# Huangying-Zhan/DF-VO

Hardware: AMD Instinct MI355X
Metric: KITTI-odom frames/sec (DF-VO per-pair tracking hot path: monodepth2 + LiteFlowNet fwd/bwd + kp selection + E/H RANSAC + scale) (higher is better)
Workload: dtype f32 (f16x3 split products: two f16 planes per operand = 22 mantissa bits, three exact products per term, fp32 accumulate; direct one- / two-channel heads exact fp32)

## Files before the change

df-vo_amd/csrc/conv_gemm_f16s.h:

```cpp
#pragma once

static inline uint32_t f16g_entry(int ky, int kx, int valid, int src, int choff) {
    return (uint32_t)ky | ((uint32_t)kx << 5) | ((uint32_t)valid << 10) | ((uint32_t)src << 11) | ((uint32_t)choff << 16);
}

typedef unsigned int u32x4 __attribute__((ext_vector_type(4)));
typedef __attribute__((address_space(4))) const u32x4 cu32x4;

template <int WP, int KSP, int TC, int PF = 3, bool RAG = false, int NP = 3>
__global__ __launch_bounds__(64 * WP * KSP) void conv_gemm_f16s_kernel(const ConvParams p) {
    extern __shared__ __attribute__((aligned(16))) float f16g_red[];

    const int t = threadIdx.x, lane = t & 63;
    const int wave = __builtin_amdgcn_readfirstlane(t >> 6);
    const int wp = wave / KSP, wk = wave % KSP;
    const int lp = lane & 31, kb = lane >> 5;
    const int M = p.N * p.Ho * p.Wo;
    const int nb = gridDim.x;
    int bid = blockIdx.x;
    {
        const int q = nb >> 3, r = nb & 7, xcd = bid & 7, k = bid >> 3;
        bid = (xcd < r ? xcd * (q + 1) : r * (q + 1) + (xcd - r) * q) + k;
    }
    const int ny = p.wf16g_cout_pad / (32 * TC);
    const int ytile = bid % ny;
    bid /= ny;
    const int m = (bid * WP + wp) * 32 + lp;
    const bool vm = m < M;
    int iy0, ix0, nimg;
    {
        const int mm = vm ? m : 0;
        nimg = mm / (p.Ho * p.Wo);
        const int rem = mm - nimg * (p.Ho * p.Wo);
        const int oy = rem / p.Wo, ox = rem - oy * p.Wo;
        iy0 = oy * p.stride - p.pad_h;
        ix0 = ox * p.stride - p.pad_w;
    }
    const int n0 = ytile * (32 * TC);
    const int S = p.f16g_steps;
    const int per = (S + KSP - 1) / KSP;
    const int s0 = wk * per < S ? wk * per : S;
    const int s1 = s0 + per < S ? s0 + per : S;

    auto pin = [](int v) { return __builtin_amdgcn_readfirstlane(v); };
    auto pin64 = [](unsigned long long v) {
        const unsigned lo = __builtin_amdgcn_readfirstlane((unsigned)v), hi = __builtin_amdgcn_readfirstlane((unsigned)(v >> 32));
        return ((unsigned long long)hi << 32) | lo;
    };
    const cu32x4* const tab = (const cu32x4*)pin64((unsigned long long)p.f16g_tab);
    const unsigned long long src0 = pin64((unsigned long long)p.src0), src1 = pin64((unsigned long long)(p.G1 ? p.src1 : p.src0));
    const int cs0 = pin(p.cs0), cs1 = pin(p.cs1), co0 = pin(p.co0), co1 = pin(p.co1), up0 = pin(p.up0);
    const int H = pin(p.H), W = pin(p.W), refl = pin(p.pad_mode == PAD_REFLECT ? 1 : 0);
    const int H0 = H >> up0, W0 = W >> up0;
    const unsigned short* const wbase = p.wf16g + ((size_t)n0 * 32 + (kb * 32 + lp) * 8);
    const size_t w_step_stride = (size_t)pin(p.wf16g_cout_pad) * 32;

    f32x4 ra[PF][2];
    unsigned rav = 0;
    h16x8 rw[PF][TC][2];
    const bool fast_addr = !refl && up0 == 0;
    int* const gtab = reinterpret_cast<int*>(f16g_red + (KSP > 1 ? WP * KSP * TC * 16 * 64 : 0));
    if (fast_addr) {
        for (int i = t; i < S * 4; i += 64 * WP * KSP) {
            const unsigned e = p.f16g_tab[i];
            const int ky = e & 31, kx = (e >> 5) & 31;
            const bool s1e = ((e >> 11) & 1u) != 0;
            gtab[2 * i] = (ky * W + kx) * (s1e ? cs1 : cs0) + (int)(e >> 16);
            gtab[2 * i + 1] = (int)(e & 0xfffu);
        }
        __syncthreads();
    }
    const int pbase0 = ((nimg * H + iy0) * W + ix0) * cs0 + co0, pbase1 = ((nimg * H + iy0) * W + ix0) * cs1 + co1;
    int nl = s0;
    u32x4 tq = tab[nl < S ? nl : S - 1];
    u32x4 gq = {0u, 0u, 0u, 0u};
    if (fast_addr) gq = *reinterpret_cast<const u32x4*>(gtab + ((nl < S ? nl : S - 1) * 4 + 2 * kb) * 2);
    auto load_step = [&](int st) {
        const int sN = nl + 1 < S ? nl + 1 : S - 1;
        if (fast_addr) {
            const u32x4 gc = gq;
            gq = *reinterpret_cast<const u32x4*>(gtab + (sN * 4 + 2 * kb) * 2);
#pragma unroll
            for (int j = 0; j < 2; ++j) {
                const int d = (int)gc[2 * j];
                const unsigned f = gc[2 * j + 1];
                const int iy = iy0 + (int)(f & 31u), ix = ix0 + (int)((f >> 5) & 31u);
                const bool s1v = ((f >> 11) & 1u) != 0;
                const bool v = vm && ((f >> 10) & 1u) && (unsigned)iy < (unsigned)H && (unsigned)ix < (unsigned)W;
                const int off = v ? (s1v ? pbase1 : pbase0) + d : (s1v ? co1 : co0);
                const unsigned long long base = s1v ? src1 : src0;
                ra[st][j] = *reinterpret_cast<const __attribute__((address_space(1))) f32x4*>(base + (long long)off * 4);
                rav = (rav & ~(1u << (2 * st + j))) | ((v ? 1u : 0u) << (2 * st + j));
            }
        } else {
        const unsigned e0 = __builtin_amdgcn_readfirstlane(tq[0]), e1 = __builtin_amdgcn_readfirstlane(tq[1]),
                       e2 = __builtin_amdgcn_readfirstlane(tq[2]), e3 = __builtin_amdgcn_readfirstlane(tq[3]);
        tq = tab[sN];
#pragma unroll
        for (int j = 0; j < 2; ++j) {
            const unsigned e = kb ? (j ? e3 : e2) : (j ? e1 : e0);
            const int ky = e & 31, kx = (e >> 5) & 31;
            const bool s1v = ((e >> 11) & 1u) != 0;
            int iy = iy0 + ky, ix = ix0 + kx;
            bool v = vm && ((e >> 10) & 1u);
            if (refl) {
                iy = reflect_idx(iy, H);
                ix = reflect_idx(ix, W);
            }
            v = v && iy >= 0 && iy < H && ix >= 0 && ix < W;
            iy = iy < 0 ? 0 : (iy >= H ? H - 1 : iy);
            ix = ix < 0 ? 0 : (ix >= W ? W - 1 : ix);
            const int pix0 = (nimg * H0 + (iy >> up0)) * W0 + (ix >> up0);
            const int pix1 = (nimg * H + iy) * W + ix;
            const int off = (s1v ? pix1 * cs1 + co1 : pix0 * cs0 + co0) + (int)(e >> 16);
            const unsigned long long base = s1v ? src1 : src0;
            ra[st][j] = *reinterpret_cast<const __attribute__((address_space(1))) f32x4*>(base + (long long)off * 4);
            rav = (rav & ~(1u << (2 * st + j))) | ((v ? 1u : 0u) << (2 * st + j));
        }
        }
        const unsigned short* g = wbase + (size_t)nl * w_step_stride;
#pragma unroll
        for (int i = 0; i < TC; ++i) {
            rw[st][i][0] = *reinterpret_cast<const h16x8*>(g + (size_t)i * 1024);
            if constexpr (NP == 3) rw[st][i][1] = *reinterpret_cast<const h16x8*>(g + (size_t)i * 1024 + 512);
        }
        ++nl;
    };

    f32x16 am[TC], ax[TC];
#pragma unroll
    for (int i = 0; i < TC; ++i)
#pragma unroll
        for (int e = 0; e < 16; ++e) am[i][e] = ax[i][e] = 0.f;
    float amax = 0.f;

#pragma unroll
    for (int d = 0; d < PF; ++d)
        if (s0 + d < s1) load_step(d);
    for (int s = s0; s < s1; s += PF) {
#pragma unroll
        for (int u = 0; u < PF; ++u) {
            if (s + u < s1) {
                h16x4 h0, l0 = {}, h1, l1 = {};
                if constexpr (NP == 3) {
                    split_f16_planes(((rav >> (2 * u)) & 1u) ? ra[u][0] : f32x4{0.f, 0.f, 0.f, 0.f}, &h0, &l0, amax);
                    split_f16_planes(((rav >> (2 * u + 1)) & 1u) ? ra[u][1] : f32x4{0.f, 0.f, 0.f, 0.f}, &h1, &l1, amax);
                } else {
                    split_f16_hi(((rav >> (2 * u)) & 1u) ? ra[u][0] : f32x4{0.f, 0.f, 0.f, 0.f}, &h0, amax);
                    split_f16_hi(((rav >> (2 * u + 1)) & 1u) ? ra[u][1] : f32x4{0.f, 0.f, 0.f, 0.f}, &h1, amax);
                }
                const h16x8 xh = __builtin_shufflevector(h0, h1, 0, 1, 2, 3, 4, 5, 6, 7);
                const h16x8 xl = __builtin_shufflevector(l0, l1, 0, 1, 2, 3, 4, 5, 6, 7);
                h16x8 wh[TC], wl[TC];
#pragma unroll
                for (int i = 0; i < TC; ++i) {
                    wh[i] = rw[u][i][0];
                    if constexpr (NP == 3) wl[i] = rw[u][i][1];
                }
                if (s + u + PF < s1) load_step(u);
                if constexpr (NP == 3) {
#pragma unroll
                    for (int i = 0; i < TC; ++i) ax[i] = __builtin_amdgcn_mfma_f32_32x32x16_f16(wh[i], xl, ax[i], 0, 0, 0);
#pragma unroll
                    for (int i = 0; i < TC; ++i) ax[i] = __builtin_amdgcn_mfma_f32_32x32x16_f16(wl[i], xh, ax[i], 0, 0, 0);
                }
#pragma unroll
                for (int i = 0; i < TC; ++i) am[i] = __builtin_amdgcn_mfma_f32_32x32x16_f16(wh[i], xh, am[i], 0, 0, 0);
            }
        }
    }
    f16s_report_clamp(amax);

    if (KSP == 1 && RAG) {
        if (!vm) return;
        float* const drow = p.dst + (size_t)m * p.dst_cs + p.dst_co;
        const float slope = p.act == ACT_LEAKY ? p.act_param : 1.f;
        f32x4 bq[4 * TC];
#pragma unroll
        for (int q = 0; q < 4 * TC; ++q) {
            const int col0 = n0 + (q >> 2) * 32 + 8 * (q & 3) + 4 * kb;
            bq[q] = *reinterpret_cast<const f32x4*>(p.bias + (col0 + 3 < p.cout_pad ? col0 : p.cout_pad - 4));
        }
#pragma unroll
        for (int q = 0; q < 4 * TC; ++q) {
            const int col0 = n0 + (q >> 2) * 32 + 8 * (q & 3) + 4 * kb;
            f32x4 x;
#pragma unroll
            for (int e = 0; e < 4; ++e) {
                const float v = am[q >> 2][4 * (q & 3) + e] + F16S_LO_UNSCALE * ax[q >> 2][4 * (q & 3) + e] + bq[q][e];
                x[e] = (v > 0.f || v != v) ? v : (p.act == ACT_RELU ? 0.f : v * slope);
            }
            if (col0 + 3 < p.cout) {
                *reinterpret_cast<f32x4*>(drow + col0) = x;
            } else {
#pragma unroll
                for (int e = 0; e < 4; ++e) {
                    if (col0 + e < p.cout)
                        drow[col0 + e] = x[e];
                    else if (col0 + e < p.dst_zero_to)
                        drow[col0 + e] = 0.f;
                }
            }
        }
        return;
    }
    if (KSP == 1) {
        ConvEpi<4 * TC> epi;
        conv_epi_init(p, epi, [&](int q) { return n0 + (q >> 2) * 32 + 8 * (q & 3) + 4 * kb; });
        conv_epi_row(p, epi, (size_t)(vm ? m : 0), vm, [&](int q) {
            f32x4 v;
#pragma unroll
            for (int e = 0; e < 4; ++e) v[e] = am[q >> 2][4 * (q & 3) + e] + F16S_LO_UNSCALE * ax[q >> 2][4 * (q & 3) + e];
            return v;
        });
        return;
    }
    float* const mine = f16g_red + (size_t)((wp * KSP + wk) * TC) * 16 * 64;
#pragma unroll
    for (int i = 0; i < TC; ++i)
#pragma unroll
        for (int e = 0; e < 16; ++e) mine[(i * 16 + e) * 64 + lane] = am[i][e] + F16S_LO_UNSCALE * ax[i][e];
    __syncthreads();
    const bool vec_ok = conv_vec_ok(p);
    for (int q = wk; q < 4 * TC; q += KSP) {
        const int i = q >> 2, g = q & 3;
        const int col0 = n0 + i * 32 + 8 * g + 4 * kb;
        const bool fastq = vec_ok && col0 + 3 < p.cout;
        f32x4 b = {0.f, 0.f, 0.f, 0.f}, r = {0.f, 0.f, 0.f, 0.f};
        if (fastq) {
            b = *reinterpret_cast<const f32x4*>(p.bias + col0);
            if (p.res && vm) r = *reinterpret_cast<const f32x4*>(p.res + (size_t)m * p.res_cs + p.res_co + col0);
        }
        f32x4 v = {0.f, 0.f, 0.f, 0.f};
        for (int z = 0; z < KSP; ++z) {
            const float* src = f16g_red + (size_t)((wp * KSP + z) * TC + i) * 16 * 64 + (4 * g) * 64 + lane;
#pragma unroll
            for (int e = 0; e < 4; ++e) v[e] = z == 0 ? src[e * 64] : v[e] + src[e * 64];
        }
        if (!vm) continue;
        if (fastq) {
            f32x4 x = v + b + r;
#pragma unroll
            for (int e = 0; e < 4; ++e) x[e] = apply_act(x[e], p.act, p.act_param);
            *reinterpret_cast<f32x4*>(p.dst + (size_t)m * p.dst_cs + p.dst_co + col0) = x;
        } else {
            conv_epilogue_quad(p, (size_t)m, col0, v, vec_ok);
        }
    }
}

size_t conv_pack_weights_f16g(const float* w, int cout, int c0, int c1, int kh, int kw, const float* fold_scale,
                              unsigned short* out) {
    const int G0 = cdiv(c0, 4), G1 = cdiv(c1, 4), G = G0 + G1, taps = kh * kw;
    const int steps = cdiv(taps * G, 4);
    const int cp = round_up(cout, 32);
    const size_t total = (size_t)steps * cp * 32;
    if (!out) return total;
    memset(out, 0, total * sizeof(unsigned short));
    const int cin = c0 + c1;
    for (int tap = 0; tap < taps; ++tap)
        for (int cg = 0; cg < G; ++cg) {
            const int g = tap * G + cg, step = g >> 2, gl = g & 3;
            for (int q = 0; q < 4; ++q) {
                int ci;
                if (cg < G0) {
                    ci = cg * 4 + q;
                    if (ci >= c0) continue;
                } else {
                    ci = (cg - G0) * 4 + q;
                    if (ci >= c1) continue;
                    ci += c0;
                }
                const int k = gl * 4 + q;
                for (int co = 0; co < cout; ++co) {
                    float v = w[((size_t)co * cin + ci) * taps + tap];
                    if (fold_scale) v *= fold_scale[co];
                    unsigned short* o = out + ((size_t)step * cp + (co & ~31)) * 32 + ((k >> 3) * 32 + (co & 31)) * 8 + (k & 7);
                    f16s_split_host(v, o, o + 512);
                }
            }
        }
    return total;
}

void conv_build_f16g_table(int c0, int c1, int kh, int kw, std::vector<uint32_t>* tab) {
    const int G0 = cdiv(c0, 4), G1 = cdiv(c1, 4), G = G0 + G1, taps = kh * kw;
    const int steps = cdiv(taps * G, 4);
    tab->assign((size_t)steps * 4, f16g_entry(0, 0, 0, 0, 0));
    for (int tap = 0; tap < taps; ++tap)
        for (int cg = 0; cg < G; ++cg)
            (*tab)[(size_t)tap * G + cg] = f16g_entry(tap / kw, tap % kw, 1, cg < G0 ? 0 : 1, cg < G0 ? cg * 4 : (cg - G0) * 4);
}

static bool conv_f16g_ok(const ConvParams& p) {
    if (!p.wf16g || !p.f16g_tab) return false;
    if (p.kh > 31 || p.kw > 31) return false;
    return true;
}

template <int WP, int KSP, int TC, int PF = 3, bool RAG = false>
static int launch_f16g_cfg(const ConvParams& p, hipStream_t stream, int cfg_id) {
    const long long M = (long long)p.N * p.Ho * p.Wo;
    dim3 grid((unsigned)(((M + 32 * WP - 1) / (32 * WP)) * (p.wf16g_cout_pad / (32 * TC))), 1, 1);
    const bool fast_addr = p.pad_mode != PAD_REFLECT && p.up0 == 0;
    const size_t lds = (KSP > 1 ? (size_t)WP * KSP * TC * 16 * 64 * sizeof(float) : 0) + (fast_addr ? (size_t)p.f16g_steps * 32 : 0);
    return with_f16_terms(p, [&](auto np) -> int {
        const auto kernel = conv_gemm_f16s_kernel<WP, KSP, TC, PF, RAG, decltype(np)::value>;
        if (lds > 48 * 1024)
            if (int rc_lds = ensure_dyn_lds((const void*)kernel, lds)) return rc_lds;
        ConvProfScope prof(p, stream, cfg_id);
        hipLaunchKernelGGL(kernel, grid, dim3(64 * WP * KSP), lds, stream, p);
        DFVO_HIP_CHECK(hipGetLastError());
        return prof.done((int)grid.x, TC, KSP * 100 + 1);
    });
}

bool conv_taps_f16s_ok(const ConvParams& p);
int launch_taps_f16s(const ConvParams& p, hipStream_t stream);

static int launch_f16g(const ConvParams& p, hipStream_t stream) {
    const long long M = (long long)p.N * p.Ho * p.Wo;
    const long long mblocks = (M + 31) / 32;
    const int nblk = p.wf16g_cout_pad / 32;
    const long long target = 2048;
    bool tc2 = (nblk % 2) == 0;
    if (tc2 && mblocks * (nblk / 2) * 8 * 2 < target && p.f16g_steps >= 64) tc2 = false;
    const long long tiles = mblocks * (tc2 ? nblk / 2 : nblk);
    int ksp = 1;
    while (ksp < (tc2 ? 8 : 16) && tiles * ksp * 2 <= target && p.f16g_steps >= 4 * ksp * 2) ksp *= 2;
    const int cfg = ksp == 1 ? 20 : 21;
    static const bool taps_on = env_flag("DFVO_TAPS", true);
    if (taps_on && ksp == 1 && conv_taps_f16s_ok(p)) {
        ConvParams pt = p;
        pt.f16s_clamp_ctr = f16s_clamp_counter();
        return launch_taps_f16s(pt, stream);
    }
    const bool rag = ksp == 1 && (p.cout % (tc2 ? 64 : 32)) != 0 && !p.res && ((p.dst_cs | p.dst_co) & 3) == 0 &&
                     p.cout_pad >= 4 && (p.act == ACT_NONE || p.act == ACT_LEAKY || p.act == ACT_RELU);
    if (rag) return tc2 ? launch_f16g_cfg<4, 1, 2, 3, true>(p, stream, cfg) : launch_f16g_cfg<4, 1, 1, 3, true>(p, stream, cfg);
    if (tc2) {
        switch (ksp) {
            case 1: return launch_f16g_cfg<4, 1, 2>(p, stream, cfg);
            case 2: return launch_f16g_cfg<2, 2, 2>(p, stream, cfg);
            case 4: return launch_f16g_cfg<1, 4, 2>(p, stream, cfg);
            default: return launch_f16g_cfg<1, 8, 2>(p, stream, cfg);
        }
    }
    switch (ksp) {
        case 1: return launch_f16g_cfg<4, 1, 1>(p, stream, cfg);
        case 2: return launch_f16g_cfg<2, 2, 1>(p, stream, cfg);
        case 4: return launch_f16g_cfg<1, 4, 1>(p, stream, cfg);
        case 8: return launch_f16g_cfg<1, 8, 1>(p, stream, cfg);
        default: return launch_f16g_cfg<1, 16, 1>(p, stream, cfg);
    }
}
```

Before: 338.1.

## Add persistent resident-grid f16 conv GEMM kernel with weights kept in registers/LDS

Adds a persistent conv GEMM kernel for short-K convolutions (2, 4, or a multiple of 3 steps). It launches a grid sized to a few blocks per CU, and each block loops over output tiles. Weights are loaded once per block into registers (when S is 2 or 4) or into LDS (when S is a multiple of 3 and cout is 32), and the activation prefetch pipeline runs across tile boundaries. This targets the per-block weight reload and launch/tail overhead on layers with small reduction depth and many output pixels. The trade-offs are higher register/LDS pressure, possible load imbalance from the fixed grid, and a simplified epilogue restricted to no-residual and simple activations.

```diff
diff --git a/df-vo_amd/csrc/conv_gemm_f16s.h b/df-vo_amd/csrc/conv_gemm_f16s.h
--- a/df-vo_amd/csrc/conv_gemm_f16s.h
+++ b/df-vo_amd/csrc/conv_gemm_f16s.h
@@ -247,6 +247,188 @@
             conv_epilogue_quad(p, (size_t)m, col0, v, vec_ok);
         }
     }
+}
+
+template <int TC, int PF, bool WREG, int NP>
+__global__ __launch_bounds__(256) void conv_gemm_f16s_res_kernel(const ConvParams p, int tiles) {
+    extern __shared__ __attribute__((aligned(16))) unsigned char f16g_res_lds[];
+    const int t = threadIdx.x, lane = t & 63;
+    const int wave = __builtin_amdgcn_readfirstlane(t >> 6);
+    const int lp = lane & 31, kb = lane >> 5;
+    const int M = p.N * p.Ho * p.Wo;
+    const int S = WREG ? PF : p.f16g_steps;
+    const int ny = p.wf16g_cout_pad / (32 * TC);
+    const int H = p.H, W = p.W, cs0 = p.cs0, co0 = p.co0;
+    auto block_of = [&](int v) {
+        const int q = tiles >> 3, r = tiles & 7, xcd = v & 7, k = v >> 3;
+        return (xcd < r ? xcd * (q + 1) : r * (q + 1) + (xcd - r) * q) + k;
+    };
+    int v = blockIdx.x;
+    const int n0 = (block_of(v) % ny) * (32 * TC);
+
+    int* const gtab = reinterpret_cast<int*>(f16g_res_lds);
+    unsigned char* const wlds = f16g_res_lds + (size_t)S * 32;
+    const unsigned te = t < S * 4 ? p.f16g_tab[t] : 0u;
+    f32x4 bq[4 * TC];
+#pragma unroll
+    for (int q = 0; q < 4 * TC; ++q) {
+        const int col0 = n0 + (q >> 2) * 32 + 8 * (q & 3) + 4 * kb;
+        bq[q] = *reinterpret_cast<const f32x4*>(p.bias + (col0 + 3 < p.cout_pad ? col0 : p.cout_pad - 4));
+    }
+    const unsigned short* const wbase = p.wf16g + ((size_t)n0 * 32 + (kb * 32 + lp) * 8);
+    const size_t w_step_stride = (size_t)p.wf16g_cout_pad * 32;
+    h16x8 rwc[WREG ? PF : 1][TC][2];
+    if constexpr (WREG) {
+#pragma unroll
+        for (int s = 0; s < PF; ++s)
+#pragma unroll
+            for (int i = 0; i < TC; ++i) {
+                rwc[s][i][0] = *reinterpret_cast<const h16x8*>(wbase + s * w_step_stride + (size_t)i * 1024);
+                if constexpr (NP == 3) rwc[s][i][1] = *reinterpret_cast<const h16x8*>(wbase + s * w_step_stride + (size_t)i * 1024 + 512);
+            }
+    } else {
+        const u32x4* const wsrc = reinterpret_cast<const u32x4*>(p.wf16g + (size_t)n0 * 32);
+        const int cps = TC * 128, nchunk = S * cps;
+        const int sstride = p.wf16g_cout_pad * 4;
+        constexpr int WB = 8;
+        for (int c0 = t; c0 < nchunk; c0 += 256 * WB) {
+            u32x4 wv[WB];
+#pragma unroll
+            for (int j = 0; j < WB; ++j) {
+                const int c = c0 + j * 256;
+                if (c < nchunk && (NP == 3 || !((c >> 6) & 1))) wv[j] = wsrc[(size_t)(c / cps) * sstride + (c % cps)];
+            }
+#pragma unroll
+            for (int j = 0; j < WB; ++j) {
+                const int c = c0 + j * 256;
+                if (c < nchunk && (NP == 3 || !((c >> 6) & 1))) *reinterpret_cast<u32x4*>(wlds + (size_t)c * 16) = wv[j];
+            }
+        }
+    }
+    for (int i = t; i < S * 4; i += 256) {
+        const unsigned e = i == t ? te : p.f16g_tab[i];
+        const int ky = e & 31, kx = (e >> 5) & 31;
+        gtab[2 * i] = (ky * W + kx) * cs0 + (int)(e >> 16);
+        gtab[2 * i + 1] = (int)(e & 0xfffu);
+    }
+    __syncthreads();
+
+    int lv = v, ls = 0;
+    bool l_live = true, l_vm = false;
+    int l_iy0 = 0, l_ix0 = 0, l_pbase = 0;
+    auto decode = [&]() {
+        const int m = ((block_of(lv) / ny) * 4 + wave) * 32 + lp;
+        l_vm = m < M;
+        const int mm = l_vm ? m : 0;
+        const int nimg = mm / (p.Ho * p.Wo);
+        const int rem = mm - nimg * (p.Ho * p.Wo);
+        const int oy = rem / p.Wo, ox = rem - oy * p.Wo;
+        l_iy0 = oy * p.stride - p.pad_h;
+        l_ix0 = ox * p.stride - p.pad_w;
+        l_pbase = ((nimg * H + l_iy0) * W + l_ix0) * cs0 + co0;
+    };
+    decode();
+    f32x4 ra[PF][2];
+    unsigned rav = 0;
+    h16x8 rw[WREG ? 1 : PF][TC][2];
+    auto load_step = [&](int st) {
+        if (l_live) {
+            const u32x4 gc = *reinterpret_cast<const u32x4*>(gtab + (ls * 4 + 2 * kb) * 2);
+#pragma unroll
+            for (int j = 0; j < 2; ++j) {
+                const int d = (int)gc[2 * j];
+                const unsigned f = gc[2 * j + 1];
+                const int iy = l_iy0 + (int)(f & 31u), ix = l_ix0 + (int)((f >> 5) & 31u);
+                const bool ok = l_vm && ((f >> 10) & 1u) && (unsigned)iy < (unsigned)H && (unsigned)ix < (unsigned)W;
+                const int off = ok ? l_pbase + d : co0;
+                ra[st][j] = *reinterpret_cast<const f32x4*>(p.src0 + off);
+                rav = (rav & ~(1u << (2 * st + j))) | ((ok ? 1u : 0u) << (2 * st + j));
+            }
+            if constexpr (!WREG) {
+                const unsigned char* g = wlds + (size_t)ls * (TC * 2048) + lane * 16;
+#pragma unroll
+                for (int i = 0; i < TC; ++i) {
+                    rw[st][i][0] = *reinterpret_cast<const h16x8*>(g + i * 2048);
+                    if constexpr (NP == 3) rw[st][i][1] = *reinterpret_cast<const h16x8*>(g + i * 2048 + 1024);
+                }
+            }
+        }
+        if (++ls == S) {
+            ls = 0;
+            lv += (int)gridDim.x;
+            l_live = lv < tiles;
+            if (l_live) decode();
+        }
+    };
+#pragma unroll
+    for (int d = 0; d < PF; ++d) load_step(d);
+
+    const float slope = p.act == ACT_LEAKY ? p.act_param : 1.f;
+    const bool full = (p.cout % (32 * TC)) == 0;
+    float amax = 0.f;
+    for (; v < tiles; v += (int)gridDim.x) {
+        f32x16 am[TC], ax[TC];
+#pragma unroll
+        for (int i = 0; i < TC; ++i)
+#pragma unroll
+            for (int e = 0; e < 16; ++e) am[i][e] = ax[i][e] = 0.f;
+        for (int s = 0; s < S; s += PF) {
+#pragma unroll
+            for (int u = 0; u < PF; ++u) {
+                h16x4 h0, l0 = {}, h1, l1 = {};
+                if constexpr (NP == 3) {
+                    split_f16_planes(((rav >> (2 * u)) & 1u) ? ra[u][0] : f32x4{0.f, 0.f, 0.f, 0.f}, &h0, &l0, amax);
+                    split_f16_planes(((rav >> (2 * u + 1)) & 1u) ? ra[u][1] : f32x4{0.f, 0.f, 0.f, 0.f}, &h1, &l1, amax);
+                } else {
+                    split_f16_hi(((rav >> (2 * u)) & 1u) ? ra[u][0] : f32x4{0.f, 0.f, 0.f, 0.f}, &h0, amax);
+                    split_f16_hi(((rav >> (2 * u + 1)) & 1u) ? ra[u][1] : f32x4{0.f, 0.f, 0.f, 0.f}, &h1, amax);
+                }
+                const h16x8 xh = __builtin_shufflevector(h0, h1, 0, 1, 2, 3, 4, 5, 6, 7);
+                const h16x8 xl = __builtin_shufflevector(l0, l1, 0, 1, 2, 3, 4, 5, 6, 7);
+                h16x8 wh[TC], wl[TC];
+#pragma unroll
+                for (int i = 0; i < TC; ++i) {
+                    wh[i] = WREG ? rwc[WREG ? u : 0][i][0] : rw[WREG ? 0 : u][i][0];
+                    if constexpr (NP == 3) wl[i] = WREG ? rwc[WREG ? u : 0][i][1] : rw[WREG ? 0 : u][i][1];
+                }
+                load_step(u);
+                if constexpr (NP == 3) {
+#pragma unroll
+                    for (int i = 0; i < TC; ++i) ax[i] = __builtin_amdgcn_mfma_f32_32x32x16_f16(wh[i], xl, ax[i], 0, 0, 0);
+#pragma unroll
+                    for (int i = 0; i < TC; ++i) ax[i] = __builtin_amdgcn_mfma_f32_32x32x16_f16(wl[i], xh, ax[i], 0, 0, 0);
+                }
+#pragma unroll
+                for (int i = 0; i < TC; ++i) am[i] = __builtin_amdgcn_mfma_f32_32x32x16_f16(wh[i], xh, am[i], 0, 0, 0);
+            }
+        }
+        const int m = ((block_of(v) / ny) * 4 + wave) * 32 + lp;
+        if (m < M) {
+            float* const drow = p.dst + (size_t)m * p.dst_cs + p.dst_co;
+#pragma unroll
+            for (int q = 0; q < 4 * TC; ++q) {
+                const int col0 = n0 + (q >> 2) * 32 + 8 * (q & 3) + 4 * kb;
+                f32x4 x;
+#pragma unroll
+                for (int e = 0; e < 4; ++e) {
+                    const float r = am[q >> 2][4 * (q & 3) + e] + F16S_LO_UNSCALE * ax[q >> 2][4 * (q & 3) + e] + bq[q][e];
+                    x[e] = (r > 0.f || r != r) ? r : (p.act == ACT_RELU ? 0.f : r * slope);
+                }
+                if (full || col0 + 3 < p.cout) {
+                    *reinterpret_cast<f32x4*>(drow + col0) = x;
+                } else {
+#pragma unroll
+                    for (int e = 0; e < 4; ++e) {
+                        if (col0 + e < p.cout)
+                            drow[col0 + e] = x[e];
+                        else if (col0 + e < p.dst_zero_to)
+                            drow[col0 + e] = 0.f;
+                    }
+                }
+            }
+        }
+    }
+    f16s_report_clamp(amax);
 }
 
 size_t conv_pack_weights_f16g(const float* w, int cout, int c0, int c1, int kh, int kw, const float* fold_scale,
@@ -318,6 +500,53 @@
 bool conv_taps_f16s_ok(const ConvParams& p);
 int launch_taps_f16s(const ConvParams& p, hipStream_t stream);
 
+static int stream_resident_cus() {
+    static int cus[64] = {};
+    int dev = 0;
+    if (hipGetDevice(&dev) != hipSuccess || dev < 0 || dev >= 64) return 256;
+    if (!cus[dev]) {
+        int n = 0;
+        cus[dev] = hipDeviceGetAttribute(&n, hipDeviceAttributeMultiprocessorCount, dev) == hipSuccess && n > 0 ? n : 256;
+    }
+    return cus[dev];
+}
+static int stream_resident_k(int rule_k) {
+    static const int k_env = [] {
+        const char* v = getenv("DFVO_STREAM_RESIDENT_K");
+        return v ? atoi(v) : 0;
+    }();
+    return k_env > 0 ? k_env : rule_k;
+}
+static int f16g_res_pf(const ConvParams& p) {
+    const bool epi_ok = !p.res && ((p.dst_cs | p.dst_co) & 3) == 0 && p.cout_pad >= 4 &&
+                        (p.act == ACT_NONE || p.act == ACT_LEAKY || p.act == ACT_RELU);
+    if (!epi_ok || p.G1 != 0 || p.pad_mode == PAD_REFLECT || p.up0 != 0) return 0;
+    const int S = p.f16g_steps;
+    if (S == 2 || S == 4) return S;
+    if (S % 3 == 0 && p.wf16g_cout_pad == 32 && (size_t)S * (32 + 2048) <= 160 * 1024) return 3;
+    return 0;
+}
+template <int TC, int PF, bool WREG>
+static int launch_f16g_res(const ConvParams& p, hipStream_t stream, int cfg_id) {
+    const long long M = (long long)p.N * p.Ho * p.Wo;
+    const int ny = p.wf16g_cout_pad / (32 * TC);
+    const int tiles = (int)((M + 127) / 128) * ny;
+    const size_t lds = (size_t)p.f16g_steps * 32 + (WREG ? 0 : (size_t)p.f16g_steps * TC * 2048);
+    const int rule_k = p.f16g_steps == 4 ? 1 : 2;
+    int grid = stream_resident_k(rule_k) * stream_resident_cus();
+    grid -= grid % (8 * ny);
+    if (grid >= tiles || grid <= 0) grid = tiles;
+    return with_f16_terms(p, [&](auto np) -> int {
+        const auto kernel = conv_gemm_f16s_res_kernel<TC, PF, WREG, decltype(np)::value>;
+        if (lds > 48 * 1024)
+            if (int rc_lds = ensure_dyn_lds((const void*)kernel, lds)) return rc_lds;
+        ConvProfScope prof(p, stream, cfg_id);
+        hipLaunchKernelGGL(kernel, dim3(grid), dim3(256), lds, stream, p, tiles);
+        DFVO_HIP_CHECK(hipGetLastError());
+        return prof.done(grid, TC, 102);
+    });
+}
+
 static int launch_f16g(const ConvParams& p, hipStream_t stream) {
     const long long M = (long long)p.N * p.Ho * p.Wo;
     const long long mblocks = (M + 31) / 32;
@@ -335,6 +564,15 @@
         pt.f16s_clamp_ctr = f16s_clamp_counter();
         return launch_taps_f16s(pt, stream);
     }
+    static const bool resident_on = env_flag("DFVO_STREAM_RESIDENT", true);
+    if (resident_on && ksp == 1) {
+        switch (f16g_res_pf(p)) {
+            case 2: return tc2 ? launch_f16g_res<2, 2, true>(p, stream, cfg) : launch_f16g_res<1, 2, true>(p, stream, cfg);
+            case 4: return tc2 ? launch_f16g_res<2, 4, true>(p, stream, cfg) : launch_f16g_res<1, 4, true>(p, stream, cfg);
+            case 3: return launch_f16g_res<1, 3, false>(p, stream, cfg);
+            default: break;
+        }
+    }
     const bool rag = ksp == 1 && (p.cout % (tc2 ? 64 : 32)) != 0 && !p.res && ((p.dst_cs | p.dst_co) & 3) == 0 &&
                      p.cout_pad >= 4 && (p.act == ACT_NONE || p.act == ACT_LEAKY || p.act == ACT_RELU);
     if (rag) return tc2 ? launch_f16g_cfg<4, 1, 2, 3, true>(p, stream, cfg) : launch_f16g_cfg<4, 1, 1, 3, true>(p, stream, cfg);
```

Measured after the change: 340.0 (median of 6 runs). No clear change (+0.6%).
